# windingwind/seal-3d

Measured on AMD Instinct MI355X. Metric: train samples/s (NGP -O step on synthetic Lego 800x800 rays), higher is better.
Workload: dtype f16; 1 GPU; configs[1]: nerf_synthetic/lego-shaped NGP -O (hashgrid L16 F2 T2^19 + ffmlp 64x2/64x3 + raymarching), 800x800 cameras, 4096 rays/step/GPU; num_rays_per_gpu=4096, parallelism=ray-sharded dp1, pretrain_steps=384, launch=hip-graph replay

## Files before the change

seal-3d_amd/csrc/ffmlp.hip:

```cpp
#include "s3d_common.hpp"
#include "sh_eval.hpp"
#include "s3d_step_tail.hpp"

namespace s3d {
namespace {

typedef _Float16 half8 __attribute__((ext_vector_type(8)));
typedef _Float16 half4 __attribute__((ext_vector_type(4)));
typedef float float16v __attribute__((ext_vector_type(16)));

enum { ACT_RELU = 0, ACT_EXP = 1, ACT_SINE = 2, ACT_SIGMOID = 3, ACT_SQUAREPLUS = 4, ACT_SOFTPLUS = 5, ACT_NONE = 6 };
constexpr float kAct = 10.0f;

__device__ __forceinline__ float act_fwd(uint32_t a, float x) {
    switch (a) {
        case ACT_RELU: return x > 0.0f ? x : 0.0f;
        case ACT_EXP: return expf(x);
        case ACT_SINE: return sinf(x);
        case ACT_SIGMOID: return 1.0f / (1.0f + expf(-x));
        case ACT_SQUAREPLUS: { float y = x * kAct; return 0.5f * (y + sqrtf(y * y + 4)) / kAct; }
        case ACT_SOFTPLUS: return logf(expf(x * kAct) + 1.0f) / kAct;
        default: return x;
    }
}
// ... 295 lines not shown
                half8 v;
                __builtin_memcpy(&v, wv, 16);
                *reinterpret_cast<half8*>(Tm + n * kMidRow + 8 * h) = v;
            }
            __builtin_amdgcn_wave_barrier();
#pragma unroll
            for (uint32_t c = 0; c < 2; c++)
                *reinterpret_cast<half8*>(mid.cin + row * 32 + 8 * (2 * h + c)) =
                    *reinterpret_cast<const half8*>(Tm + n * kMidRow + 8 * (2 * h + c));
            __builtin_amdgcn_wave_barrier();
            continue;
        }
        if (rgb_head) {
            if (h == 0) {
#pragma unroll
                for (uint32_t c = 0; c < 3; c++) {
                    const _Float16 v = (_Float16)act_fwd_t<OACT>(out_act, (float)(_Float16)o[c]);
                    rgb_head[row * 3 + c] = (float)(_Float16)(1.0f / (1.0f + expf(-(float)v)));
                }
            }
            continue;
        }
        _Float16* orow = out + row * 16;
#pragma unroll
        for (uint32_t q = 0; q < 2; q++) {
            half4 v;
#pragma unroll
            for (uint32_t e = 0; e < 4; e++) v[e] = (_Float16)act_fwd_t<OACT>(out_act, (float)(_Float16)o[4 * q + e]);
            st4(orow + 8 * q + 4 * h, v);
        }
    }
}

#ifndef S3D_PAIR_WAVES
#define S3D_PAIR_WAVES 8
#endif
constexpr uint32_t kPairWaves = S3D_PAIR_WAVES;
struct PairNets {
    const _Float16* Ws;
    const _Float16* Wc;
    uint32_t nl_s, nl_c;
    const _Float16* enc_c;
};
template <uint32_t KPX>
__device__ __forceinline__ float16v pair_network(const half8* a0, uint32_t NH, const half8 (&b0)[KPX], uint32_t lane) {
    constexpr uint32_t MB = 2, KS = 4, nf0 = MB * KPX;
    float16v acc[MB];
    half8 bf[KS];
#pragma unroll
    for (uint32_t m = 0; m < MB; m++) acc[m] = zero16();
#pragma unroll
    for (uint32_t s = 0; s < KPX; s++) {
#pragma unroll
        for (uint32_t m = 0; m < MB; m++) acc[m] = mfma(a0[(m * KPX + s) * 64 + lane], b0[s], acc[m]);
    }
    for (uint32_t layer = 0;; layer++) {
#pragma unroll
        for (uint32_t m = 0; m < MB; m++)
#pragma unroll
            for (uint32_t r = 0; r < 16; r += 2) {
                const half2p v = relu2(cvt2(acc[m][r], acc[m][r + 1]));
                bf[2 * m + (r >> 3)][r & 7] = v[0];
                bf[2 * m + (r >> 3)][(r & 7) + 1] = v[1];
            }
        if (layer == NH) break;
        const half8* a = a0 + (size_t)(nf0 + layer * MB * KS) * 64;
#pragma unroll
        for (uint32_t m = 0; m < MB; m++) {
            acc[m] = zero16();
#pragma unroll
            for (uint32_t s = 0; s < KS; s++) acc[m] = mfma(a[(m * KS + s) * 64 + lane], bf[s], acc[m]);
        }
    }
    float16v o = zero16();
    const half8* a = a0 + (size_t)(nf0 + NH * MB * KS) * 64;
#pragma unroll
    for (uint32_t s = 0; s < KS; s++) o = mfma(a[s * 64 + lane], bf[s], o);
    return o;
}
template <bool SEAL>
__global__ void __launch_bounds__(kPairWaves * 64) k_ffmlp_ngp_pair(const _Float16* __restrict__ X, const PairNets nets, uint32_t B,
                                                                   uint32_t in_layout, const int32_t* __restrict__ n_valid,
                                                                   float* __restrict__ rgb_head, const MidFwd mid) {
    constexpr uint32_t W = 64, MB = 2, KS = 4, KP = 2, IN = 32;
    constexpr uint32_t KPC = SEAL ? 4 : 2, INC = 16 * KPC;
    constexpr uint32_t kRow = SEAL ? 72 : kMidRow;
    extern __shared__ __attribute__((aligned(16))) unsigned char smem_raw[];
    half8* frags = reinterpret_cast<half8*>(smem_raw);
    const uint32_t lane = threadIdx.x & 63, wave = threadIdx.x >> 6;
    const uint32_t n = lane & 31, h = lane >> 5;
    const uint32_t NHs = nets.nl_s - 1, NHc = nets.nl_c - 1;
    constexpr uint32_t nf0 = MB * KP, nf0c = MB * KPC;
    const uint32_t tot_s = nf0 + NHs * MB * KS + KS, tot_c = nf0c + NHc * MB * KS + KS;
    _Float16* Tm = reinterpret_cast<_Float16*>(frags + (size_t)(tot_s + tot_c) * 64) + (size_t)wave * 32 * kRow;

#pragma unroll 1
    for (uint32_t f0 = wave; f0 < tot_s + tot_c; f0 += kPairWaves) {
        const bool second = f0 >= tot_s;
        const uint32_t f = second ? f0 - tot_s : f0, NH = second ? NHc : NHs;
        const uint32_t in_w = second ? INC : IN, ks0 = second ? KPC : KP, n0 = MB * ks0;
        const _Float16* Wt = second ? nets.Wc : nets.Ws;
        const _Float16* w_hid = Wt + (size_t)W * in_w;
        const _Float16* w_last = w_hid + (size_t)NH * W * W;
        const uint32_t nfh = NH * MB * KS;
        const _Float16* r;
        bool live = true;
        if (f < n0) {
            const uint32_t mblk = f / ks0, s = f % ks0;
            r = Wt + (size_t)(mblk * 32 + n) * in_w + 16 * s;
        } else if (f < n0 + nfh) {
            const uint32_t g = f - n0, k = g / (MB * KS), mblk = (g / KS) % MB, s = g % KS;
            r = w_hid + (size_t)k * W * W + (size_t)(mblk * 32 + n) * W + 16 * s;
        } else {
            const uint32_t s = f - n0 - nfh;
            live = n < 16;
            r = w_last + (size_t)(live ? n : 0) * W + 16 * s;
        }
        frags[f0 * 64 + lane] = live ? load_bfrag_rowmajor(r, 0, h) : zero_half8();
    }
    __syncthreads();

    const uint32_t ntiles = valid_rows(B, n_valid) / 32;
    const uint32_t tstride = gridDim.x * kPairWaves;
    constexpr uint32_t NE = SEAL ? 8 : 1;
    half8 bin[KP];
    float dir[3] = {0.0f, 0.0f, 0.0f};
    uint32_t enc[NE];
    auto request = [&](uint32_t t, half8 (&dst)[KP], float (&d)[3], uint32_t (&e)[NE]) {
        const size_t r = (size_t)t * 32 + n;
#pragma unroll
        for (uint32_t s = 0; s < KP; s++) dst[s] = load_bfrag_input(X, in_layout, B, IN, r, s, h);
        d[0] = mid.dirs[r * 3]; d[1] = mid.dirs[r * 3 + 1]; d[2] = mid.dirs[r * 3 + 2];
        if constexpr (SEAL) {
#pragma unroll
            for (uint32_t l = 0; l < NE; l++)
                e[l] = *reinterpret_cast<const uint32_t*>(nets.enc_c + ((size_t)(8 * h + l) * B + r) * 2);
        }
    };
    uint32_t tile = blockIdx.x * kPairWaves + wave;
#pragma unroll
    for (uint32_t l = 0; l < NE; l++) enc[l] = 0u;
    if (tile < ntiles) request(tile, bin, dir, enc);
    for (; tile < ntiles; tile += tstride) {
        const size_t row = (size_t)tile * 32 + n;
        half8 bnx[KP];
        float dnx[3] = {0.0f, 0.0f, 0.0f};
        uint32_t enx[NE];
#pragma unroll
        for (uint32_t l = 0; l < NE; l++) enx[l] = 0u;
        if (tile + tstride < ntiles) request(tile + tstride, bnx, dnx, enx);
        const float16v o = pair_network<KP>(frags, NHs, bin, lane);
#pragma unroll
        for (uint32_t s = 0; s < KP; s++) bin[s] = bnx[s];
        const float dx = dir[0], dy = dir[1], dz = dir[2];
        dir[0] = dnx[0]; dir[1] = dnx[1]; dir[2] = dnx[2];
#pragma unroll
        for (uint32_t q = 0; q < 2; q++)
#pragma unroll
            for (uint32_t e = 0; e < 4; e++) {
                const uint32_t f = 8 * q + 4 * h + e;
                const _Float16 v = (_Float16)o[4 * q + e];
                if (f == 0) {
                    mid.sigma[row] = expf((float)v);
                    if (mid.h0) mid.h0[row] = v;
                } else {
                    Tm[n * kRow + 15 + f] = v;
                }
            }
        if constexpr (SEAL) {
#pragma unroll
            for (uint32_t l = 0; l < NE; l++) {
                const uint32_t c0 = 31 + 2 * (8 * h + l);
                _Float16 lo, hi;
                const uint16_t lo16 = (uint16_t)(enc[l] & 0xFFFFu), hi16 = (uint16_t)(enc[l] >> 16);
                __builtin_memcpy(&lo, &lo16, 2);
// ... 13 lines not shown
            half8 vlo, vhi;
#pragma unroll
            for (uint32_t i = 0; i < 8; i++) { vlo[i] = (_Float16)sh[i]; vhi[i] = (_Float16)sh[8 + i]; }
            uint32_t wl[4], wh[4], wv[4];
            __builtin_memcpy(wl, &vlo, 16);
            __builtin_memcpy(wh, &vhi, 16);
#pragma unroll
            for (uint32_t i = 0; i < 4; i++) wv[i] = h ? wh[i] : wl[i];
            half8 v;
            __builtin_memcpy(&v, wv, 16);
            *reinterpret_cast<half8*>(Tm + n * kRow + 8 * h) = v;
        }
        __builtin_amdgcn_wave_barrier();
        half8 bc[KPC];
#pragma unroll
        for (uint32_t s = 0; s < KPC; s++) bc[s] = load_bfrag_rowmajor(Tm + n * kRow, s, h);
        if (mid.cin) {
            constexpr uint32_t PC = INC / 16;
#pragma unroll
            for (uint32_t c = 0; c < PC; c++)
                *reinterpret_cast<half8*>(mid.cin + row * INC + 8 * (PC * h + c)) =
                    *reinterpret_cast<const half8*>(Tm + n * kRow + 8 * (PC * h + c));
        }
        __builtin_amdgcn_wave_barrier();
        const float16v oc = pair_network<KPC>(frags + (size_t)tot_s * 64, NHc, bc, lane);
        if (h == 0) {
#pragma unroll
            for (uint32_t c = 0; c < 3; c++) {
                const _Float16 v = (_Float16)oc[c];
                rgb_head[row * 3 + c] = (float)(_Float16)(1.0f / (1.0f + expf(-(float)v)));
            }
        }
    }
}

template <int W, int ACT>
__global__ void __launch_bounds__(256) k_ffmlp_dgrad(const _Float16* __restrict__ grad, const _Float16* __restrict__ Wt,
                                                     const _Float16* __restrict__ fwd, uint32_t B, uint32_t in_dim,
                                                     uint32_t out_dim, uint32_t n_layers, uint32_t act,
                                                     _Float16* __restrict__ bwd, _Float16* __restrict__ grad_inputs,
                                                     const int32_t* __restrict__ n_valid) {
    constexpr uint32_t MB = W / 32, KS = W / 16;
    extern __shared__ __attribute__((aligned(16))) unsigned char smem_raw[];
    half8* frags = reinterpret_cast<half8*>(smem_raw);

    const uint32_t lane = threadIdx.x & 63, wave = threadIdx.x >> 6;
    const uint32_t n = lane & 31, h = lane >> 5;
    const uint32_t NH = n_layers - 1;
    const uint32_t IMB = (in_dim + 31) / 32;
    const uint32_t nfl = MB, nfh = NH * MB * KS, nf0 = grad_inputs ? IMB * KS : 0, total = nfl + nfh + nf0;
    const _Float16* w_hid = Wt + (size_t)W * in_dim;
    const _Float16* w_last = w_hid + (size_t)NH * W * W;

    for (uint32_t f = wave; f < total; f += 4) {
        half8 v;
        if (f < nfl) {
            const uint32_t i = f * 32 + n;
#pragma unroll
            for (uint32_t j = 0; j < 8; j++) {
                const uint32_t k = kperm(h, j);
                v[j] = (k < out_dim) ? w_last[(size_t)k * W + i] : (_Float16)0.0f;
            }
        } else if (f < nfl + nfh) {
            const uint32_t g = f - nfl, k = g / (MB * KS), mblk = (g / KS) % MB, s = g % KS;
            const _Float16* wk = w_hid + (size_t)k * W * W;
#pragma unroll
// ... 239 lines not shown
typedef __fp16 fp16x4 __attribute__((__vector_size__(4 * sizeof(__fp16))));

template <int NS>
__device__ __forceinline__ void transpose_store(_Float16* __restrict__ T, const half8 (&bf)[NS], uint32_t ksteps,
                                                uint32_t n, uint32_t h) {
#pragma unroll
    for (uint32_t s = 0; s < (uint32_t)NS; s++)
        if (s < ksteps) {
            half4 lo, hi;
#pragma unroll
            for (uint32_t j = 0; j < 4; j++) { lo[j] = bf[s][j]; hi[j] = bf[s][4 + j]; }
            _Float16* row = T + n * kTRow + 16 * s + 4 * h;
            *reinterpret_cast<half4*>(row) = lo;
            *reinterpret_cast<half4*>(row + 8) = hi;
        }
}
__device__ __forceinline__ half8 transpose_load(const _Float16* __restrict__ T, uint32_t blk, uint32_t s, uint32_t fl,
                                                uint32_t h, uint32_t nfeat) {
    const uint32_t i = fl & 15, g1 = fl >> 4;
    const _Float16* p = T + (16 * s + 8 * h + i / 4) * kTRow + 32 * blk + 16 * g1 + 4 * (i % 4);
    typedef __attribute__((address_space(3))) fp16x4 lds_fp16x4;
    const fp16x4 a = __builtin_amdgcn_ds_read_tr16_b64_v4f16((lds_fp16x4*)p);
    const fp16x4 b = __builtin_amdgcn_ds_read_tr16_b64_v4f16((lds_fp16x4*)(p + 4 * kTRow));
    half8 v;
#pragma unroll
    for (uint32_t j = 0; j < 4; j++) { v[j] = (_Float16)a[j]; v[4 + j] = (_Float16)b[j]; }
    if (blk * 32 + fl >= nfeat) {
#pragma unroll
        for (uint32_t j = 0; j < 8; j++) v[j] = (_Float16)0.0f;
    }
    return v;
}

template <uint32_t MBLK, uint32_t NBLK, uint32_t THREADS, uint32_t NPL, typename Get>
__device__ __forceinline__ void flush_matrix(float* __restrict__ red, float* __restrict__ partial, uint32_t matrix, uint32_t wave,
                                             uint32_t n, uint32_t h, Get&& get) {
    constexpr uint32_t kPlane = kWgradPad * kWgradPad;
    __syncthreads();
    float* mine = red + (size_t)wave * kPlane;
    if (wave < NPL) {
#pragma unroll
        for (uint32_t mo = 0; mo < MBLK; mo++)
#pragma unroll
            for (uint32_t ni = 0; ni < NBLK; ni++) {
                const float16v v = get(mo, ni);
#pragma unroll
                for (uint32_t r = 0; r < 16; r++) mine[(mo * 32 + (r & 3) + 8 * (r >> 2) + 4 * h) * kWgradPad + ni * 32 + n] = v[r];
            }
    }
    __syncthreads();
    float* dst = partial + ((size_t)matrix * gridDim.x + blockIdx.x) * kPlane;
    for (uint32_t i = threadIdx.x; i < kPlane; i += THREADS) {
        const uint32_t o = i / kWgradPad, c = i % kWgradPad;
        float v = 0.0f;
        if (o < MBLK * 32 && c < NBLK * 32) {
            v = red[i];
#pragma unroll
            for (uint32_t p = 1; p < NPL; p++) v += red[p * kPlane + i];
        }
        dst[i] = v;
    }
}

template <typename F, uint32_t... I>
__device__ __forceinline__ void static_for_impl(F&& f, std::integer_sequence<uint32_t, I...>) {
    (f(std::integral_constant<uint32_t, I>{}), ...);
}
template <uint32_t N, typename F>
__device__ __forceinline__ void static_for(F&& f) { static_for_impl(f, std::make_integer_sequence<uint32_t, N>{}); }

#ifdef S3D_FFMLP_PROF
#ifndef S3D_FFMLP_PROF_BLOCK
#define S3D_FFMLP_PROF_BLOCK 7
#endif
__device__ unsigned long long s3d_ffmlp_prof[2][1024];
#define DUO_STAMP() do { if (prof_on && prof_k < 1024) s3d_ffmlp_prof[role][prof_k++] = __builtin_amdgcn_s_memtime(); } while (0)
#else
#define DUO_STAMP() do { } while (0)
#endif
__device__ __forceinline__ void duo_barrier() {
    __builtin_amdgcn_fence(__ATOMIC_RELEASE, "workgroup", "local");
    __builtin_amdgcn_s_barrier();
    __builtin_amdgcn_fence(__ATOMIC_ACQUIRE, "workgroup", "local");
}
template <int W, int NH, int IMB, int ACT, int KS0T, int NC, int NG>
__global__ void __launch_bounds__((NC + NG) * 64) k_ffmlp_backward_duo(const _Float16* __restrict__ grad, const _Float16* __restrict__ X,
                                                            const _Float16* __restrict__ Wt, uint32_t B, uint32_t in_dim,
                                                            uint32_t out_dim, uint32_t act, _Float16* __restrict__ grad_inputs,
                                                            float* __restrict__ partial, uint32_t in_layout,
                                                            const int32_t* __restrict__ n_valid,
                                                            const float* __restrict__ d_rgb, const float* __restrict__ rgb_head,
                                                            const MidBwd midb) {
    constexpr uint32_t MB = W / 32, KS = W / 16, NS = NH + 2;
    extern __shared__ __attribute__((aligned(16))) unsigned char smem_raw[];
    const uint32_t lane = threadIdx.x & 63;
    const uint32_t wave = __builtin_amdgcn_readfirstlane(threadIdx.x >> 6);
    static_assert(NC % NG == 0, "every weight-gradient wave serves the same number of compute waves");
    constexpr uint32_t NR = NC / NG;
    const uint32_t role = wave < (uint32_t)NC ? 0u : 1u;
    const uint32_t pair = role == 0 ? wave : wave - (uint32_t)NC;
    const uint32_t n = lane & 31, h = lane >> 5;
    const uint32_t KS0 = KS0T ? (uint32_t)KS0T : in_dim / 16;
    const uint32_t nf_f0 = MB * KS0, nf_fh = NH * MB * KS;
    const uint32_t nf_bl = MB, nf_bh = NH * MB * KS, nf_b0 = grad_inputs ? IMB * KS : 0;
#ifdef S3D_FFMLP_PROF
    uint32_t prof_k = 0;
    const bool prof_on = NH == S3D_FFMLP_PROF && blockIdx.x == S3D_FFMLP_PROF_BLOCK && pair == 0 && lane == 0;
#endif
    const uint32_t nfrag = nf_f0 + nf_fh + nf_bl + nf_bh + nf_b0;
    half8* frags = reinterpret_cast<half8*>(smem_raw);
    half8* ff0 = frags;
    half8* ffh = ff0 + (size_t)nf_f0 * 64;
    half8* fbl = ffh + (size_t)nf_fh * 64;
    half8* fbh = fbl + (size_t)nf_bl * 64;
    half8* fb0 = fbh + (size_t)nf_bh * 64;
    _Float16* tiles = reinterpret_cast<_Float16*>(frags + (size_t)nfrag * 64);
    constexpr uint32_t kTile = kTRows * kTRow;
    const _Float16* w_hid = Wt + (size_t)W * in_dim;
    const _Float16* w_last = w_hid + (size_t)NH * W * W;

    for (uint32_t f = wave; f < nfrag; f += NC + NG) {
        half8 v;
        if (f < nf_f0) {
            const uint32_t mblk = f / KS0, s = f % KS0;
            const _Float16* r = Wt + (size_t)(mblk * 32 + n) * in_dim + 16 * s;
#pragma unroll
            for (uint32_t j = 0; j < 8; j++) v[j] = r[kperm(h, j)];
        } else if (f < nf_f0 + nf_fh) {
            const uint32_t g = f - nf_f0, k = g / (MB * KS), mblk = (g / KS) % MB, s = g % KS;
            const _Float16* r = w_hid + (size_t)k * W * W + (size_t)(mblk * 32 + n) * W + 16 * s;
#pragma unroll
            for (uint32_t j = 0; j < 8; j++) v[j] = r[kperm(h, j)];
        } else if (f < nf_f0 + nf_fh + nf_bl) {
            const uint32_t i = (f - nf_f0 - nf_fh) * 32 + n;
#pragma unroll
            for (uint32_t j = 0; j < 8; j++) {
                const uint32_t k = kperm(h, j);
                v[j] = (k < out_dim) ? w_last[(size_t)k * W + i] : (_Float16)0.0f;
            }
        } else if (f < nf_f0 + nf_fh + nf_bl + nf_bh) {
            const uint32_t g = f - nf_f0 - nf_fh - nf_bl, k = g / (MB * KS), mblk = (g / KS) % MB, s = g % KS;
            const _Float16* wk = w_hid + (size_t)k * W * W;
#pragma unroll
            for (uint32_t j = 0; j < 8; j++) v[j] = wk[(size_t)(16 * s + kperm(h, j)) * W + mblk * 32 + n];
        } else {
            const uint32_t g = f - nf_f0 - nf_fh - nf_bl - nf_bh, mblk = g / KS, s = g % KS;
            const uint32_t i = mblk * 32 + n;
#pragma unroll
            for (uint32_t j = 0; j < 8; j++)
                v[j] = (i < in_dim) ? Wt[(size_t)(16 * s + kperm(h, j)) * in_dim + i] : (_Float16)0.0f;
        }
        frags[f * 64 + lane] = v;
    }
    __syncthreads();

    const uint32_t ntiles = valid_rows(B, n_valid) / 32;
    const uint32_t first = blockIdx.x * NC, stride = gridDim.x * NC;
    const uint32_t nit = ntiles > first ? (ntiles - first - 1) / stride + 1 : 0;
    auto tile_of = [&](uint32_t c, uint32_t i) { return first + c + i * stride; };
    auto slot_of = [&](uint32_t c, uint32_t i, uint32_t st) { return tiles + (size_t)c * 4 * kTile + (size_t)((i * NS + st) & 1u) * 2 * kTile; };

    if (role == 0) {
        for (uint32_t i = 0; i < nit; i++) {
            const uint32_t tile = tile_of(pair, i);
            const bool live = tile < ntiles;
            const size_t row = (size_t)(live ? tile : 0) * 32 + n;
            half8 xf[4];
            half8 gf;
            half8 a[NH + 1][KS];
            float16v acc[MB];
            half8 G[KS];
            DUO_STAMP();
            if (live) {
#pragma unroll
                for (uint32_t s = 0; s < 4; s++)
                    if (s < KS0) xf[s] = load_bfrag_input(X, in_layout, B, in_dim, row, s, h);
                if (d_rgb) {
#pragma unroll
                    for (uint32_t j = 0; j < 8; j++) gf[j] = (_Float16)0.0f;
                    if (h == 0) {
#pragma unroll
                        for (uint32_t c = 0; c < 3; c++) {
                            const float y = rgb_head[row * 3 + c];
                            gf[c] = (_Float16)((float)(_Float16)d_rgb[row * 3 + c] * (y * (1.0f - y)));
                        }
                    }
                } else if (midb.g_cin) {
// ... 80 lines not shown
                        for (uint32_t m = 0; m < MB; m++) {
                            acc[m] = zero16();
#pragma unroll
                            for (uint32_t s = 0; s < KS; s++) acc[m] = mfma(wf[(m * KS + s) * 64 + lane], G[s], acc[m]);
                        }
                    } else {
                        transpose_store<4>(T + kTile, xf, KS0, n, h);
                        if (grad_inputs) {
#pragma unroll
                            for (uint32_t m = 0; m < (uint32_t)IMB; m++) {
                                float16v gi = zero16();
#pragma unroll
                                for (uint32_t s = 0; s < KS; s++) gi = mfma(fb0[(m * KS + s) * 64 + lane], G[s], gi);
#pragma unroll
                                for (uint32_t q = 0; q < 4; q++) {
                                    const uint32_t feat = m * 32 + 8 * q + 4 * h;
                                    if (feat < in_dim) {
                                        half4 v;
#pragma unroll
                                        for (uint32_t e = 0; e < 4; e++) v[e] = (_Float16)gi[4 * q + e];
                                        store_grad_input(grad_inputs, in_layout, B, in_dim, row, feat, v);
                                    }
                                }
                            }
                        }
                    }
                }
                DUO_STAMP();
                duo_barrier();
                DUO_STAMP();
            }
        }
        if (nit) duo_barrier();
    } else {
        float16v dw0[MB][IMB], dwh[NH > 0 ? NH : 1][MB][MB], dwl[MB];
#pragma unroll
        for (uint32_t p = 0; p < MB; p++) {
#pragma unroll
            for (uint32_t q = 0; q < (uint32_t)IMB; q++) dw0[p][q] = zero16();
#pragma unroll
            for (uint32_t k = 0; k < (uint32_t)NH; k++)
#pragma unroll
                for (uint32_t q = 0; q < MB; q++) dwh[k][p][q] = zero16();
            dwl[p] = zero16();
        }
        auto consume = [&](uint32_t i, auto stc) {
            constexpr uint32_t st = decltype(stc)::value;
#pragma unroll 1
            for (uint32_t j = 0; j < NR; j++) {
            const uint32_t cw = pair + j * (uint32_t)NG;
            if (tile_of(cw, i) >= ntiles) continue;
            const _Float16* T = slot_of(cw, i, st);
            const _Float16* TXs = T + kTile;
            if constexpr (st == 0) {
#pragma unroll
                for (uint32_t s = 0; s < 2; s++) {
                    const half8 af = transpose_load(T, 0, s, n, h, 16);
#pragma unroll
                    for (uint32_t ni = 0; ni < MB; ni++) dwl[ni] = mfma(af, transpose_load(TXs, ni, s, n, h, W), dwl[ni]);
                }
            } else if constexpr (st <= (uint32_t)NH) {
                constexpr uint32_t k = NH - (st - 1);
#pragma unroll
                for (uint32_t s = 0; s < 2; s++) {
                    half8 bfr[MB];
#pragma unroll
// ... 7 lines not shown
                }
            } else {
#pragma unroll
                for (uint32_t s = 0; s < 2; s++) {
                    half8 bfr[IMB];
#pragma unroll
                    for (uint32_t ni = 0; ni < (uint32_t)IMB; ni++) bfr[ni] = transpose_load(TXs, ni, s, n, h, in_dim);
#pragma unroll
                    for (uint32_t mo = 0; mo < MB; mo++) {
                        const half8 af = transpose_load(T, mo, s, n, h, W);
#pragma unroll
                        for (uint32_t ni = 0; ni < (uint32_t)IMB; ni++) dw0[mo][ni] = mfma(af, bfr[ni], dw0[mo][ni]);
                    }
                }
            }
            }
        };
        for (uint32_t i = 0; i < nit; i++) {
            DUO_STAMP();
            if (i > 0) consume(i - 1, std::integral_constant<uint32_t, NS - 1>{});
            DUO_STAMP();
            duo_barrier();
            static_for<NS - 1>([&](auto stc) {
                DUO_STAMP();
                consume(i, stc);
                DUO_STAMP();
                duo_barrier();
            });
        }
        if (nit) {
            consume(nit - 1, std::integral_constant<uint32_t, NS - 1>{});
            duo_barrier();
        }
        float* red = reinterpret_cast<float*>(smem_raw);
        flush_matrix<MB, IMB, (NC + NG) * 64, NG>(red, partial, 0, pair, n, h, [&](auto mo, auto ni) { return dw0[mo][ni]; });
#pragma unroll
        for (uint32_t k = 0; k < (uint32_t)NH; k++)
            flush_matrix<MB, MB, (NC + NG) * 64, NG>(red, partial, 1 + k, pair, n, h, [&](auto mo, auto ni) { return dwh[k][mo][ni]; });
        flush_matrix<1, MB, (NC + NG) * 64, NG>(red, partial, NH + 1, pair, n, h, [&](auto mo, auto ni) { (void)mo; return dwl[ni]; });
        return;
    }
    float* red = reinterpret_cast<float*>(smem_raw);
    const float16v none = zero16();
    flush_matrix<MB, IMB, (NC + NG) * 64, NG>(red, partial, 0, NG + pair, n, h, [&](auto, auto) { return none; });
#pragma unroll
    for (uint32_t k = 0; k < (uint32_t)NH; k++) flush_matrix<MB, MB, (NC + NG) * 64, NG>(red, partial, 1 + k, NG + pair, n, h, [&](auto, auto) { return none; });
    flush_matrix<1, MB, (NC + NG) * 64, NG>(red, partial, NH + 1, NG + pair, n, h, [&](auto, auto) { return none; });
}

constexpr uint32_t kWgradBlocks = 256;
inline uint32_t wgrad_blocks(uint32_t W) { return W > 64 ? 128u : kWgradBlocks; }
}
bool ffmlp_native_shape(uint32_t in_dim, uint32_t W, uint32_t n_layers = 2);
size_t ffmlp_generic_min_workspace(uint32_t in_dim, uint32_t W, uint32_t n_layers);
int ffmlp_generic_forward(const _Float16* X, const _Float16* Wt, uint32_t B, uint32_t in_dim, uint32_t W, uint32_t n_layers, uint32_t act,
                          uint32_t out_act, _Float16* acts, bool training, _Float16* out, hipStream_t st);
int ffmlp_generic_backward(const _Float16* grad, const _Float16* X, const _Float16* Wt, const _Float16* fwd, uint32_t B, uint32_t in_dim,
                           uint32_t W, uint32_t n_layers, uint32_t act, _Float16* bwd, _Float16* grad_inputs, _Float16* grad_weights,
                           bool accumulate, float* found_inf, float* workspace, size_t workspace_bytes, hipStream_t st);
namespace {

struct FwdArgs {
    const _Float16 *X, *Wt;
    uint32_t B, in_dim, out_dim, n_layers, act, out_act;
    _Float16 *fwd, *out;
    uint32_t in_layout;
    hipStream_t st;
};
struct FwdOpts {
    const int32_t* n_valid;
    float* rgb_out;
    MidFwd mid;
    _Float16* scratch;
};
struct BwdArgs {
    const _Float16 *grad, *X, *Wt, *fwd;
    uint32_t B, in_dim, out_dim, n_layers, act;
    _Float16 *bwd, *grad_inputs, *grad_weights;
    float* partial;
    size_t partial_bytes;
// ... 77 lines not shown
        S3D_REQUIRE(plan.n < kMaxMlpLayers, "ffmlp_backward: too many layers for an input wider than the hidden width");
        plan.layer[0].Fi = (uint32_t)W; plan.layer[0].x_ld = in_dim; plan.layer[0].x_col0 = 0u; plan.layer[0].w_ld = in_dim;
        plan.layer[plan.n] = WgradLayer{bwd + NH * BW, X, 1u, 0u, (uint32_t)W, in_dim - (uint32_t)W, (uint32_t)W, in_dim, (uint32_t)W, in_dim};
        plan.n++;
    }
    uint32_t nblk = div_up<uint32_t>(ntiles, 4);
    if (nblk > wgrad_blocks(W)) nblk = wgrad_blocks(W);
    hipLaunchKernelGGL((k_ffmlp_wgrad<W>), dim3(nblk, plan.n), dim3(256), 0, a.st, plan, B, a.partial, o.n_valid);
    const uint32_t widest = (uint32_t)W > in_dim ? (uint32_t)W : in_dim;
    hipLaunchKernelGGL(k_ffmlp_wgrad_reduce, dim3(div_up<uint32_t>(W * widest * kReduceSplit, 256), plan.n), dim3(256), 0, a.st, plan, nblk,
                       (const float*)a.partial, a.grad_weights, a.accumulate, o.found_inf, wgrad_pad(W));
    return check_launch("ffmlp_backward");
}

inline uint32_t fused_max_hidden(uint32_t W) { return W == 64 ? 2u : 3u; }

inline bool fused_backward_supported(uint32_t in_dim, uint32_t out_dim, uint32_t W, uint32_t n_layers, uint32_t act) {
    if (!ffmlp_native_shape(in_dim, W)) return false;
    return (W == 32 || W == 64) && in_dim % 16 == 0 && in_dim >= 16 && in_dim <= 64 && out_dim >= 1 && out_dim <= 16 &&
           n_layers >= 2 && n_layers - 1 <= fused_max_hidden(W) && act != ACT_SINE;
}

template <int W, int NH, int IMB, int ACT, int KS0T>
int launch_backward_fused_k(const BwdArgs& a, const BwdOpts& o) {
    const uint32_t B = a.B, in_dim = a.in_dim;
    constexpr uint32_t MB = W / 32, KS = W / 16;
    constexpr int NC = 6, NG = 2;
    const uint32_t nfrag = MB * (in_dim / 16) + NH * MB * KS + MB + NH * MB * KS + (a.grad_inputs ? IMB * KS : 0);
    const uint32_t ntiles = B / 32;
    uint32_t nblk = div_up<uint32_t>(ntiles, 4);
    if (nblk > kWgradBlocks) nblk = kWgradBlocks;
    auto smem_for = [&](uint32_t owners, uint32_t slots, uint32_t planes) {
        size_t v = (size_t)nfrag * 64 * sizeof(half8) + (size_t)owners * slots * 2 * kTRows * kTRow * sizeof(_Float16);
        if (v < planes * kWgradPad * kWgradPad * sizeof(float)) v = planes * kWgradPad * kWgradPad * sizeof(float);
        return v;
    };
    const size_t smem = smem_for(NC, 2, NG);
    S3D_REQUIRE(smem <= 160 * 1024, "ffmlp_backward: wave mix %dx%d needs %zu bytes of LDS", NC, NG, smem);
    static std::atomic<uint64_t> attr_devs{0};
    int dev;
    if (device_needs_setup(attr_devs, &dev)) {
        S3D_HIP(hipFuncSetAttribute(reinterpret_cast<const void*>(&k_ffmlp_backward_duo<W, NH, IMB, ACT, KS0T, NC, NG>),
                                    hipFuncAttributeMaxDynamicSharedMemorySize, 160 * 1024));
        device_setup_done(attr_devs, dev);
    }
    hipLaunchKernelGGL((k_ffmlp_backward_duo<W, NH, IMB, ACT, KS0T, NC, NG>), dim3(nblk), dim3((NC + NG) * 64), smem, a.st, a.grad, a.X,
                       a.Wt, B, in_dim, a.out_dim, a.act, a.grad_inputs, a.partial, a.in_layout, o.n_valid, o.d_rgb, o.rgb_in, o.mid);
    WgradPlan plan;
    memset(&plan, 0, sizeof(plan));
    plan.n = NH + 2;
    plan.layer[0] = WgradLayer{nullptr, nullptr, 0u, 0u, (uint32_t)W, in_dim, 0u};
    for (uint32_t m = 0; m < (uint32_t)NH; m++)
        plan.layer[1 + m] = WgradLayer{nullptr, nullptr, 0u, 0u, (uint32_t)W, (uint32_t)W, (uint32_t)(W * in_dim + m * W * W)};
    plan.layer[NH + 1] = WgradLayer{nullptr, nullptr, 0u, 0u, 16u, (uint32_t)W, (uint32_t)(W * in_dim + NH * W * W)};
    if (a.accumulate != 2u)
        hipLaunchKernelGGL(k_ffmlp_wgrad_reduce, dim3(div_up<uint32_t>(W * W * kReduceSplit, 256), plan.n), dim3(256), 0, a.st, plan, nblk,
                           (const float*)a.partial, a.grad_weights, a.accumulate, o.found_inf, kWgradPad);
    return check_launch("ffmlp_backward (fused)");
}

template <int W>
int launch_backward_fused(const BwdArgs& a, const BwdOpts& o) {
    const uint32_t NH = a.n_layers - 1, in_dim = a.in_dim, IMB = (in_dim + 31) / 32, act = a.act;
#define S3D_FUSED_K(NHV, IMBV, ACTV, KSV) launch_backward_fused_k<W, NHV, IMBV, ACTV, KSV>(a, o)
#define S3D_FUSED(NHV, IMBV)                                                                                  \
    (act == ACT_RELU ? (in_dim == 32u * IMBV ? S3D_FUSED_K(NHV, IMBV, ACT_RELU, 2 * IMBV) : S3D_FUSED_K(NHV, IMBV, ACT_RELU, 0)) \
                     : S3D_FUSED_K(NHV, IMBV, -1, 0))
// ... 210 lines not shown
                    "[n, B, W], row-major inputs, no heads, no n_valid", hidden_dim, input_dim);
        return ffmlp_generic_backward(a.grad, a.X, a.Wt, a.fwd, B, input_dim, hidden_dim, num_layers, activation, a.bwd, a.grad_inputs,
                                      a.grad_weights, accumulate != 0, found_inf, a.partial, a.partial_bytes, a.st);
    }
    const bool fused = !forward_buffer;
    S3D_REQUIRE(!fused || fused_backward_supported(input_dim, 16, hidden_dim, num_layers, activation),
                "ffmlp_backward: this network shape needs forward_buffer/backward_buffer (s3d_ffmlp_fused_backward_supported)");
    switch (hidden_dim) {
        case 64: return fused ? launch_backward_fused<64>(a, o) : launch_backward<64>(a, o);
        case 128: return launch_backward<128>(a, o);
        default: return fused ? launch_backward_fused<32>(a, o) : launch_backward<32>(a, o);
    }
}

S3D_EXPORT int s3d_ffmlp_fused_backward_supported(uint32_t input_dim, uint32_t output_dim, uint32_t hidden_dim,
                                                  uint32_t num_layers, uint32_t activation) {
    return fused_backward_supported(input_dim, output_dim, hidden_dim, num_layers, activation) ? 1 : 0;
}

S3D_EXPORT int s3d_ffmlp_allocate_splitk(size_t n) { (void)n; return S3D_OK; }
S3D_EXPORT int s3d_ffmlp_free_splitk(void) { return S3D_OK; }

#ifdef S3D_FFMLP_PROF
S3D_EXPORT int s3d_debug_ffmlp_prof_read(unsigned long long* dst, int clear) {
    if (hipDeviceSynchronize() != hipSuccess) return S3D_ERR_HIP;
    if (hipMemcpyFromSymbol(dst, HIP_SYMBOL(s3d_ffmlp_prof), sizeof(unsigned long long) * 2 * 1024) != hipSuccess) return S3D_ERR_HIP;
    if (clear) {
        void* p = nullptr;
        if (hipGetSymbolAddress(&p, HIP_SYMBOL(s3d_ffmlp_prof)) != hipSuccess) return S3D_ERR_HIP;
        if (hipMemset(p, 0, sizeof(unsigned long long) * 2 * 1024) != hipSuccess) return S3D_ERR_HIP;
    }
    return S3D_OK;
}
#endif
```

Before: 695.7 million samples/s.

## Batch weight staging loads, transpose backward weights from LDS, and vectorize wgrad flush

The pair forward kernel now issues weight-fragment loads in batches of six per wave, and only after the first input tile request, so those global loads overlap instead of serialising. The fused backward kernel copies the raw weights coalesced into the tile slots in LDS. It then builds the transposed backward fragments from LDS rather than doing strided global gathers. The wgrad flush stores every per-pair plane once and sums them with a single barrier and float4 accesses, replacing the old per-matrix double-barrier flush. In exchange the flush needs more LDS, and the code adds profiling edge timestamps that compile only under a debug macro.

```diff
diff --git a/seal-3d_amd/csrc/ffmlp.hip b/seal-3d_amd/csrc/ffmlp.hip
--- a/seal-3d_amd/csrc/ffmlp.hip
+++ b/seal-3d_amd/csrc/ffmlp.hip
@@ -351,6 +351,20 @@
     }
 }
 
+#ifdef S3D_FFMLP_PROF
+#ifndef S3D_FFMLP_PROF_BLOCK
+#define S3D_FFMLP_PROF_BLOCK 7
+#endif
+__device__ unsigned long long s3d_ffmlp_prof[2][1024];
+#define DUO_STAMP() do { if (prof_on && prof_k < 1024) s3d_ffmlp_prof[role][prof_k++] = __builtin_amdgcn_s_memtime(); } while (0)
+__device__ unsigned long long s3d_ffmlp_edge[2][8];
+#define EDGE_STAMP(kernel, k) do { if (edge_on) { s3d_ffmlp_edge[kernel][k] = __builtin_amdgcn_s_memtime(); \
+                                                  s3d_ffmlp_edge[kernel][4 + (k)] = __builtin_amdgcn_s_memrealtime(); } } while (0)
+#else
+#define DUO_STAMP() do { } while (0)
+#define EDGE_STAMP(kernel, k) do { } while (0)
+#endif
+
 #ifndef S3D_PAIR_WAVES
 #define S3D_PAIR_WAVES 8
 #endif
@@ -412,32 +426,10 @@
     constexpr uint32_t nf0 = MB * KP, nf0c = MB * KPC;
     const uint32_t tot_s = nf0 + NHs * MB * KS + KS, tot_c = nf0c + NHc * MB * KS + KS;
     _Float16* Tm = reinterpret_cast<_Float16*>(frags + (size_t)(tot_s + tot_c) * 64) + (size_t)wave * 32 * kRow;
-
-#pragma unroll 1
-    for (uint32_t f0 = wave; f0 < tot_s + tot_c; f0 += kPairWaves) {
-        const bool second = f0 >= tot_s;
-        const uint32_t f = second ? f0 - tot_s : f0, NH = second ? NHc : NHs;
-        const uint32_t in_w = second ? INC : IN, ks0 = second ? KPC : KP, n0 = MB * ks0;
-        const _Float16* Wt = second ? nets.Wc : nets.Ws;
-        const _Float16* w_hid = Wt + (size_t)W * in_w;
-        const _Float16* w_last = w_hid + (size_t)NH * W * W;
-        const uint32_t nfh = NH * MB * KS;
-        const _Float16* r;
-        bool live = true;
-        if (f < n0) {
-            const uint32_t mblk = f / ks0, s = f % ks0;
-            r = Wt + (size_t)(mblk * 32 + n) * in_w + 16 * s;
-        } else if (f < n0 + nfh) {
-            const uint32_t g = f - n0, k = g / (MB * KS), mblk = (g / KS) % MB, s = g % KS;
-            r = w_hid + (size_t)k * W * W + (size_t)(mblk * 32 + n) * W + 16 * s;
-        } else {
-            const uint32_t s = f - n0 - nfh;
-            live = n < 16;
-            r = w_last + (size_t)(live ? n : 0) * W + 16 * s;
-        }
-        frags[f0 * 64 + lane] = live ? load_bfrag_rowmajor(r, 0, h) : zero_half8();
-    }
-    __syncthreads();
+#ifdef S3D_FFMLP_PROF
+    const bool edge_on = blockIdx.x == S3D_FFMLP_PROF_BLOCK && threadIdx.x == 0;
+#endif
+    EDGE_STAMP(1, 0);
 
     const uint32_t ntiles = valid_rows(B, n_valid) / 32;
     const uint32_t tstride = gridDim.x * kPairWaves;
@@ -460,6 +452,47 @@
 #pragma unroll
     for (uint32_t l = 0; l < NE; l++) enc[l] = 0u;
     if (tile < ntiles) request(tile, bin, dir, enc);
+
+    constexpr uint32_t kStageBatch = 6;
+    const uint32_t wave_u = __builtin_amdgcn_readfirstlane(wave);
+#pragma unroll 1
+    for (uint32_t base = wave_u; base < tot_s + tot_c; base += kStageBatch * kPairWaves) {
+        half8 v[kStageBatch];
+#pragma unroll
+        for (uint32_t t = 0; t < kStageBatch; t++) {
+            const uint32_t f0 = base + t * kPairWaves;
+            if (f0 >= tot_s + tot_c) continue;
+            const bool second = f0 >= tot_s;
+            const uint32_t f = second ? f0 - tot_s : f0, NH = second ? NHc : NHs;
+            const uint32_t in_w = second ? INC : IN, ks0 = second ? KPC : KP, n0 = MB * ks0;
+            const _Float16* Wt = second ? nets.Wc : nets.Ws;
+            const _Float16* w_hid = Wt + (size_t)W * in_w;
+            const _Float16* w_last = w_hid + (size_t)NH * W * W;
+            const uint32_t nfh = NH * MB * KS;
+            const _Float16* r;
+            bool live = true;
+            if (f < n0) {
+                const uint32_t mblk = f / ks0, s = f % ks0;
+                r = Wt + (size_t)(mblk * 32 + n) * in_w + 16 * s;
+            } else if (f < n0 + nfh) {
+                const uint32_t g = f - n0, k = g / (MB * KS), mblk = (g / KS) % MB, s = g % KS;
+                r = w_hid + (size_t)k * W * W + (size_t)(mblk * 32 + n) * W + 16 * s;
+            } else {
+                const uint32_t s = f - n0 - nfh;
+                live = n < 16;
+                r = w_last + (size_t)(live ? n : 0) * W + 16 * s;
+            }
+            v[t] = live ? load_bfrag_rowmajor(r, 0, h) : zero_half8();
+        }
+#pragma unroll
+        for (uint32_t t = 0; t < kStageBatch; t++) {
+            const uint32_t f0 = base + t * kPairWaves;
+            if (f0 < tot_s + tot_c) frags[f0 * 64 + lane] = v[t];
+        }
+    }
+    __syncthreads();
+    EDGE_STAMP(1, 1);
+
     for (; tile < ntiles; tile += tstride) {
         const size_t row = (size_t)tile * 32 + n;
         half8 bnx[KP];
@@ -539,6 +572,8 @@
             }
         }
     }
+    EDGE_STAMP(1, 2);
+    EDGE_STAMP(1, 3);
 }
 
 template <int W, int ACT>
@@ -844,33 +879,35 @@
     return v;
 }
 
-template <uint32_t MBLK, uint32_t NBLK, uint32_t THREADS, uint32_t NPL, typename Get>
-__device__ __forceinline__ void flush_matrix(float* __restrict__ red, float* __restrict__ partial, uint32_t matrix, uint32_t wave,
-                                             uint32_t n, uint32_t h, Get&& get) {
-    constexpr uint32_t kPlane = kWgradPad * kWgradPad;
-    __syncthreads();
-    float* mine = red + (size_t)wave * kPlane;
-    if (wave < NPL) {
-#pragma unroll
-        for (uint32_t mo = 0; mo < MBLK; mo++)
-#pragma unroll
-            for (uint32_t ni = 0; ni < NBLK; ni++) {
-                const float16v v = get(mo, ni);
-#pragma unroll
-                for (uint32_t r = 0; r < 16; r++) mine[(mo * 32 + (r & 3) + 8 * (r >> 2) + 4 * h) * kWgradPad + ni * 32 + n] = v[r];
-            }
-    }
-    __syncthreads();
-    float* dst = partial + ((size_t)matrix * gridDim.x + blockIdx.x) * kPlane;
-    for (uint32_t i = threadIdx.x; i < kPlane; i += THREADS) {
-        const uint32_t o = i / kWgradPad, c = i % kWgradPad;
-        float v = 0.0f;
-        if (o < MBLK * 32 && c < NBLK * 32) {
-            v = red[i];
-#pragma unroll
-            for (uint32_t p = 1; p < NPL; p++) v += red[p * kPlane + i];
-        }
-        dst[i] = v;
+template <int W, int NH, int IMB> struct FlushPlanes {
+    static constexpr uint32_t kOff0 = 0;
+    static constexpr uint32_t kOffH = (uint32_t)W * 32u * (uint32_t)IMB;
+    static constexpr uint32_t kOffL = kOffH + (uint32_t)NH * W * W;
+    static constexpr uint32_t kSet = kOffL + 32u * (uint32_t)W;
+};
+template <uint32_t MBLK, uint32_t NBLK, typename Get>
+__device__ __forceinline__ void flush_store(float* __restrict__ mine, uint32_t n, uint32_t h, Get&& get) {
+#pragma unroll
+    for (uint32_t mo = 0; mo < MBLK; mo++)
+#pragma unroll
+        for (uint32_t ni = 0; ni < NBLK; ni++) {
+            const float16v v = get(mo, ni);
+#pragma unroll
+            for (uint32_t r = 0; r < 16; r++) mine[(mo * 32 + (r & 3) + 8 * (r >> 2) + 4 * h) * (NBLK * 32) + ni * 32 + n] = v[r];
+        }
+}
+template <uint32_t PITCH, uint32_t THREADS, uint32_t NPL>
+__device__ __forceinline__ void flush_sum(const float* __restrict__ red, uint32_t set_stride, float* __restrict__ partial, uint32_t matrix,
+                                          uint32_t Fo, uint32_t Fi) {
+    typedef float f4v __attribute__((ext_vector_type(4)));
+    float* dst = partial + ((size_t)matrix * gridDim.x + blockIdx.x) * (kWgradPad * kWgradPad);
+    const uint32_t per_row = Fi / 4;
+    for (uint32_t q = threadIdx.x; q < Fo * per_row; q += THREADS) {
+        const uint32_t o = q / per_row, c = (q - o * per_row) * 4;
+        f4v v = *reinterpret_cast<const f4v*>(red + o * PITCH + c);
+#pragma unroll
+        for (uint32_t p = 1; p < NPL; p++) v += *reinterpret_cast<const f4v*>(red + p * set_stride + o * PITCH + c);
+        *reinterpret_cast<f4v*>(dst + o * kWgradPad + c) = v;
     }
 }
 
@@ -881,15 +918,6 @@
 template <uint32_t N, typename F>
 __device__ __forceinline__ void static_for(F&& f) { static_for_impl(f, std::make_integer_sequence<uint32_t, N>{}); }
 
-#ifdef S3D_FFMLP_PROF
-#ifndef S3D_FFMLP_PROF_BLOCK
-#define S3D_FFMLP_PROF_BLOCK 7
-#endif
-__device__ unsigned long long s3d_ffmlp_prof[2][1024];
-#define DUO_STAMP() do { if (prof_on && prof_k < 1024) s3d_ffmlp_prof[role][prof_k++] = __builtin_amdgcn_s_memtime(); } while (0)
-#else
-#define DUO_STAMP() do { } while (0)
-#endif
 __device__ __forceinline__ void duo_barrier() {
     __builtin_amdgcn_fence(__ATOMIC_RELEASE, "workgroup", "local");
     __builtin_amdgcn_s_barrier();
@@ -904,6 +932,7 @@
                                                             const float* __restrict__ d_rgb, const float* __restrict__ rgb_head,
                                                             const MidBwd midb) {
     constexpr uint32_t MB = W / 32, KS = W / 16, NS = NH + 2;
+    using FL = FlushPlanes<W, NH, IMB>;
     extern __shared__ __attribute__((aligned(16))) unsigned char smem_raw[];
     const uint32_t lane = threadIdx.x & 63;
     const uint32_t wave = __builtin_amdgcn_readfirstlane(threadIdx.x >> 6);
@@ -918,7 +947,9 @@
 #ifdef S3D_FFMLP_PROF
     uint32_t prof_k = 0;
     const bool prof_on = NH == S3D_FFMLP_PROF && blockIdx.x == S3D_FFMLP_PROF_BLOCK && pair == 0 && lane == 0;
+    const bool edge_on = prof_on && role == 0;
 #endif
+    EDGE_STAMP(0, 0);
     const uint32_t nfrag = nf_f0 + nf_fh + nf_bl + nf_bh + nf_b0;
     half8* frags = reinterpret_cast<half8*>(smem_raw);
     half8* ff0 = frags;
@@ -929,42 +960,82 @@
     _Float16* tiles = reinterpret_cast<_Float16*>(frags + (size_t)nfrag * 64);
     constexpr uint32_t kTile = kTRows * kTRow;
     const _Float16* w_hid = Wt + (size_t)W * in_dim;
-    const _Float16* w_last = w_hid + (size_t)NH * W * W;
-
-    for (uint32_t f = wave; f < nfrag; f += NC + NG) {
-        half8 v;
-        if (f < nf_f0) {
-            const uint32_t mblk = f / KS0, s = f % KS0;
-            const _Float16* r = Wt + (size_t)(mblk * 32 + n) * in_dim + 16 * s;
-#pragma unroll
-            for (uint32_t j = 0; j < 8; j++) v[j] = r[kperm(h, j)];
-        } else if (f < nf_f0 + nf_fh) {
-            const uint32_t g = f - nf_f0, k = g / (MB * KS), mblk = (g / KS) % MB, s = g % KS;
-            const _Float16* r = w_hid + (size_t)k * W * W + (size_t)(mblk * 32 + n) * W + 16 * s;
-#pragma unroll
-            for (uint32_t j = 0; j < 8; j++) v[j] = r[kperm(h, j)];
-        } else if (f < nf_f0 + nf_fh + nf_bl) {
-            const uint32_t i = (f - nf_f0 - nf_fh) * 32 + n;
-#pragma unroll
-            for (uint32_t j = 0; j < 8; j++) {
-                const uint32_t k = kperm(h, j);
-                v[j] = (k < out_dim) ? w_last[(size_t)k * W + i] : (_Float16)0.0f;
-            }
-        } else if (f < nf_f0 + nf_fh + nf_bl + nf_bh) {
-            const uint32_t g = f - nf_f0 - nf_fh - nf_bl, k = g / (MB * KS), mblk = (g / KS) % MB, s = g % KS;
-            const _Float16* wk = w_hid + (size_t)k * W * W;
-#pragma unroll
-            for (uint32_t j = 0; j < 8; j++) v[j] = wk[(size_t)(16 * s + kperm(h, j)) * W + mblk * 32 + n];
-        } else {
-            const uint32_t g = f - nf_f0 - nf_fh - nf_bl - nf_bh, mblk = g / KS, s = g % KS;
-            const uint32_t i = mblk * 32 + n;
-#pragma unroll
-            for (uint32_t j = 0; j < 8; j++)
-                v[j] = (i < in_dim) ? Wt[(size_t)(16 * s + kperm(h, j)) * in_dim + i] : (_Float16)0.0f;
-        }
-        frags[f * 64 + lane] = v;
+
+    constexpr uint32_t THREADS = (NC + NG) * 64;
+    constexpr uint32_t kMaxIn = KS0T ? 16u * KS0T : 32u * IMB;
+    constexpr uint32_t kRawMax = W * kMaxIn + NH * W * W + 16 * W;
+    static_assert(kRawMax * sizeof(_Float16) <= (size_t)NC * 4 * kTile * sizeof(_Float16), "the weight copy lives in the tile slots");
+    constexpr uint32_t kRawTrips = (kRawMax / 8 + THREADS - 1) / THREADS;
+    constexpr uint32_t kFwdTrips = (MB * (kMaxIn / 16) + NH * MB * KS + NC + NG - 1) / (NC + NG);
+    constexpr uint32_t kTrTrips = (MB + NH * MB * KS + IMB * KS + NC + NG - 1) / (NC + NG);
+    _Float16* raw = tiles;
+    {
+        const uint32_t nchunk = (W * in_dim + NH * W * W + 16 * W) / 8, nfwd = nf_f0 + nf_fh;
+        half8 rv[kRawTrips], fv[kFwdTrips];
+#pragma unroll
+        for (uint32_t t = 0; t < kRawTrips; t++) {
+            const uint32_t c = threadIdx.x + t * THREADS;
+            if (c < nchunk) rv[t] = *reinterpret_cast<const half8*>(Wt + (size_t)c * 8);
+        }
+#pragma unroll
+        for (uint32_t t = 0; t < kFwdTrips; t++) {
+            const uint32_t f = wave + t * (NC + NG);
+            if (f >= nfwd) continue;
+            const _Float16* r;
+            if (f < nf_f0) {
+                const uint32_t mblk = f / KS0, s = f % KS0;
+                r = Wt + (size_t)(mblk * 32 + n) * in_dim + 16 * s;
+            } else {
+                const uint32_t g = f - nf_f0, k = g / (MB * KS), mblk = (g / KS) % MB, s = g % KS;
+                r = w_hid + (size_t)k * W * W + (size_t)(mblk * 32 + n) * W + 16 * s;
+            }
+            fv[t] = load_bfrag_rowmajor(r, 0, h);
+        }
+#pragma unroll
+        for (uint32_t t = 0; t < kRawTrips; t++) {
+            const uint32_t c = threadIdx.x + t * THREADS;
+            if (c < nchunk) *reinterpret_cast<half8*>(raw + (size_t)c * 8) = rv[t];
+        }
+#pragma unroll
+        for (uint32_t t = 0; t < kFwdTrips; t++) {
+            const uint32_t f = wave + t * (NC + NG);
+            if (f < nfwd) frags[f * 64 + lane] = fv[t];
+        }
     }
     __syncthreads();
+    {
+        const _Float16* r_hid = raw + (size_t)W * in_dim;
+        const _Float16* r_last = r_hid + (size_t)NH * W * W;
+        half8* fb = fbl;
+#pragma unroll
+        for (uint32_t t = 0; t < kTrTrips; t++) {
+            const uint32_t f = wave + t * (NC + NG);
+            if (f >= nf_bl + nf_bh + nf_b0) continue;
+            half8 v;
+            if (f < nf_bl) {
+                const uint32_t i = f * 32 + n;
+#pragma unroll
+                for (uint32_t j = 0; j < 8; j++) {
+                    const uint32_t k = kperm(h, j);
+                    v[j] = (k < out_dim) ? r_last[k * W + i] : (_Float16)0.0f;
+                }
+            } else if (f < nf_bl + nf_bh) {
+                const uint32_t g = f - nf_bl, k = g / (MB * KS), mblk = (g / KS) % MB, s = g % KS;
+                const _Float16* wk = r_hid + (size_t)k * W * W;
+#pragma unroll
+                for (uint32_t j = 0; j < 8; j++) v[j] = wk[(16 * s + kperm(h, j)) * W + mblk * 32 + n];
+            } else {
+                const uint32_t g = f - nf_bl - nf_bh, mblk = g / KS, s = g % KS;
+                const uint32_t i = mblk * 32 + n;
+#pragma unroll
+                for (uint32_t j = 0; j < 8; j++)
+                    v[j] = (i < in_dim) ? raw[(16 * s + kperm(h, j)) * in_dim + i] : (_Float16)0.0f;
+            }
+            fb[f * 64 + lane] = v;
+        }
+    }
+    __syncthreads();
+    EDGE_STAMP(0, 1);
 
     const uint32_t ntiles = valid_rows(B, n_valid) / 32;
     const uint32_t first = blockIdx.x * NC, stride = gridDim.x * NC;
@@ -1111,6 +1182,7 @@
             }
         }
         if (nit) duo_barrier();
+        EDGE_STAMP(0, 2);
     } else {
         float16v dw0[MB][IMB], dwh[NH > 0 ? NH : 1][MB][MB], dwl[MB];
 #pragma unroll
@@ -1184,20 +1256,22 @@
             consume(nit - 1, std::integral_constant<uint32_t, NS - 1>{});
             duo_barrier();
         }
-        float* red = reinterpret_cast<float*>(smem_raw);
-        flush_matrix<MB, IMB, (NC + NG) * 64, NG>(red, partial, 0, pair, n, h, [&](auto mo, auto ni) { return dw0[mo][ni]; });
+        float* mine = reinterpret_cast<float*>(smem_raw) + (size_t)pair * FL::kSet;
+        flush_store<MB, IMB>(mine + FL::kOff0, n, h, [&](auto mo, auto ni) { return dw0[mo][ni]; });
 #pragma unroll
         for (uint32_t k = 0; k < (uint32_t)NH; k++)
-            flush_matrix<MB, MB, (NC + NG) * 64, NG>(red, partial, 1 + k, pair, n, h, [&](auto mo, auto ni) { return dwh[k][mo][ni]; });
-        flush_matrix<1, MB, (NC + NG) * 64, NG>(red, partial, NH + 1, pair, n, h, [&](auto mo, auto ni) { (void)mo; return dwl[ni]; });
-        return;
-    }
-    float* red = reinterpret_cast<float*>(smem_raw);
-    const float16v none = zero16();
-    flush_matrix<MB, IMB, (NC + NG) * 64, NG>(red, partial, 0, NG + pair, n, h, [&](auto, auto) { return none; });
-#pragma unroll
-    for (uint32_t k = 0; k < (uint32_t)NH; k++) flush_matrix<MB, MB, (NC + NG) * 64, NG>(red, partial, 1 + k, NG + pair, n, h, [&](auto, auto) { return none; });
-    flush_matrix<1, MB, (NC + NG) * 64, NG>(red, partial, NH + 1, NG + pair, n, h, [&](auto, auto) { return none; });
+            flush_store<MB, MB>(mine + FL::kOffH + k * W * W, n, h, [&](auto mo, auto ni) { return dwh[k][mo][ni]; });
+        flush_store<1, MB>(mine + FL::kOffL, n, h, [&](auto mo, auto ni) { (void)mo; return dwl[ni]; });
+    }
+    __syncthreads();
+    {
+        const float* red = reinterpret_cast<const float*>(smem_raw);
+        flush_sum<IMB * 32, THREADS, NG>(red + FL::kOff0, FL::kSet, partial, 0, W, in_dim);
+#pragma unroll
+        for (uint32_t k = 0; k < (uint32_t)NH; k++) flush_sum<W, THREADS, NG>(red + FL::kOffH + k * W * W, FL::kSet, partial, 1 + k, W, W);
+        flush_sum<W, THREADS, NG>(red + FL::kOffL, FL::kSet, partial, NH + 1, 16, W);
+    }
+    EDGE_STAMP(0, 3);
 }
 
 constexpr uint32_t kWgradBlocks = 256;
@@ -1341,7 +1415,8 @@
     if (nblk > kWgradBlocks) nblk = kWgradBlocks;
     auto smem_for = [&](uint32_t owners, uint32_t slots, uint32_t planes) {
         size_t v = (size_t)nfrag * 64 * sizeof(half8) + (size_t)owners * slots * 2 * kTRows * kTRow * sizeof(_Float16);
-        if (v < planes * kWgradPad * kWgradPad * sizeof(float)) v = planes * kWgradPad * kWgradPad * sizeof(float);
+        const size_t flush = (size_t)planes * FlushPlanes<W, NH, IMB>::kSet * sizeof(float);
+        if (v < flush) v = flush;
         return v;
     };
     const size_t smem = smem_for(NC, 2, NG);
@@ -1618,4 +1693,14 @@
     }
     return S3D_OK;
 }
+S3D_EXPORT int s3d_debug_ffmlp_edge_read(unsigned long long* dst, int clear) {
+    if (hipDeviceSynchronize() != hipSuccess) return S3D_ERR_HIP;
+    if (hipMemcpyFromSymbol(dst, HIP_SYMBOL(s3d_ffmlp_edge), sizeof(unsigned long long) * 2 * 8) != hipSuccess) return S3D_ERR_HIP;
+    if (clear) {
+        void* p = nullptr;
+        if (hipGetSymbolAddress(&p, HIP_SYMBOL(s3d_ffmlp_edge)) != hipSuccess) return S3D_ERR_HIP;
+        if (hipMemset(p, 0, sizeof(unsigned long long) * 2 * 8) != hipSuccess) return S3D_ERR_HIP;
+    }
+    return S3D_OK;
+}
 #endif
```

Measured after the change: 698.8 million samples/s (median of 4 runs). No clear change (+0.4%).
